# HunterJ-Lin/WSOVOD

Hardware: AMD Instinct MI355X
Metric: images/sec (512 proposals/img) WSR_18_DC5 fwd+bwd at 1/2/4/8 MI355X (higher is better)
Workload: dtype bf16 / fp16 + MX fp8 (the parity forward with the res4 / res5 convs and fc1 / fc2 on fp16 hi*hi + block-scaled e4m3 cross terms -- two v_mfma_f32_32x32x16_f16 + one v_mfma_scale_f32_32x32x64_f8f6f4 per 32x32x32 tile --, bf16x2 three-product forward elsewhere; plain bf16 backward; fp32 accumulation

## Files before the change

### include/wsovod_hip.h

```cpp
#ifndef WSOVOD_HIP_H_
#define WSOVOD_HIP_H_

#ifdef __cplusplus
extern "C" {
#endif

typedef void* wsovod_stream_t;

typedef enum {
  WSOVOD_OK = 0,
  WSOVOD_ERR_INVALID_ARGUMENT = 1,
  WSOVOD_ERR_HIP = 2,
  WSOVOD_ERR_UNSUPPORTED = 3
} wsovod_status;

typedef enum { WSOVOD_F32 = 0, WSOVOD_BF16 = 1, WSOVOD_BF16X2 = 2, WSOVOD_BF16X2P = 3, WSOVOD_F16MX = 4 } wsovod_dtype;
typedef enum { WSOVOD_NCHW = 0, WSOVOD_NHWC = 1 } wsovod_layout;

const char* wsovod_last_error(void);
int wsovod_abi_version(void);

typedef struct {
  const char* name;
  long long launches;
// ... 248 lines not shown

int wsovod_mask_transpose(const void* dy, long long lddy, const void* y, long long ldy, int in_dtype,
                          int M, int N, float scale, void* dA, long long ldda, void* dAt, long long ldt,
                          int out_dtype, wsovod_stream_t stream);
int wsovod_mask_transpose_colsum(const void* dy, long long lddy, const void* y, long long ldy, int in_dtype,
                                 int M, int N, float scale, void* dA, long long ldda, void* dAt, long long ldt,
                                 int out_dtype, float* colsum, wsovod_stream_t stream);
int wsovod_mask_transpose_ex(const void* dy, long long lddy, int dy_dtype, const void* y, long long ldy, int y_dtype, int M,
                             int N, float scale, void* dA, long long ldda, void* dAt, long long ldt, int out_dtype,
                             float* colsum, wsovod_stream_t stream);
int wsovod_bf16x2_encode(const float* src, long long ld_src, int rows, int cols, void* dst, long long ld_dst,
                         wsovod_stream_t stream);
int wsovod_bf16x2_decode(const void* src, long long ld_src, int rows, int cols, float* dst, long long ld_dst,
                         wsovod_stream_t stream);
int wsovod_mask_bf16x2(const float* dy, long long lddy, const void* y, long long ldy, int y_dtype, int M, int N, float scale,
                       void* dA_x2, long long ld_x2, void* dA_hi, long long ld_hi, float* colsum, wsovod_stream_t stream);
int wsovod_bf16x2_encode_t(const float* src, long long ld_src, int N, int K, void* dst, long long ld_dst,
                           wsovod_stream_t stream);
int wsovod_f16mx_to_f32(const void* src, long long ld_src, int rows, int cols, float* dst, long long ld_dst,
                        wsovod_stream_t stream);
int wsovod_f16mx_range(const void* src, long long ld, int rows, int cols, long long* counters, wsovod_stream_t stream);
int wsovod_stem_conv1_x2(const unsigned char* img, const int* sizes, const float* mean_host, const float* std_host, int N,
                         int Hp, int Wp, const void* w32x2, const float* bias, void* out, wsovod_stream_t stream);
int wsovod_add_group_rows(const void* x, long long ldx, int dtype, const int* row_group, const float* add,
                          long long ld_add, int M, int N, void* out, long long ldo, wsovod_stream_t stream);
int wsovod_scale_rows(const float* x, long long ldx, const float* row_scale, int R, int C, void* out,
                      long long ldo, int out_dtype, wsovod_stream_t stream);

int wsovod_data_aware_forward(const float* gap, int N, int C, const float* W1, const float* b1, int Hd,
                              const float* W2, const float* b2, int P, const float* E, int F, float* h1,
                              float* h2, float* daf, wsovod_stream_t stream);
int wsovod_data_aware_backward(const float* ddaf, int N, const float* gap, int C, const float* W2,
                               const float* E, int F, const float* h1, int Hd, const float* h2, int P,
                               float* dW1, float* db1, float* dW2, float* db2, float* dE,
                               float* scratch , wsovod_stream_t stream);

#ifdef __cplusplus
}
#endif
#endif
```

### wsovod_amd/_lib.py

```python
import ctypes as C
import os

import torch

_HERE = os.path.dirname(os.path.abspath(__file__))
LIB_PATH = os.path.join(_HERE, "lib", "libwsovod_hip.so")

F32, BF16, BF16X2, BF16X2P, F16MX = 0, 1, 2, 3, 4
NCHW, NHWC = 0, 1


class ConvGeom(C.Structure):
    _fields_ = [(n, C.c_int) for n in
                ("n_img", "H", "W", "Cin", "Ho", "Wo", "KH", "KW", "stride", "pad", "dil", "pool")]


class GemmDesc(C.Structure):
    _fields_ = [
        ("dtype_in", C.c_int), ("M", C.c_int), ("N", C.c_int), ("K", C.c_int),
        ("A", C.c_void_p), ("lda", C.c_longlong),
        ("B", C.c_void_p), ("ldb", C.c_longlong),
        ("C", C.c_void_p), ("ldc", C.c_longlong), ("dtype_c", C.c_int),
        ("Ct", C.c_void_p), ("ldct", C.c_longlong), ("dtype_ct", C.c_int),
        ("alpha", C.c_float),
# ... 21 lines not shown
_P, _I, _L, _F = C.c_void_p, C.c_int, C.c_longlong, C.c_float
ABI_VERSION = 9

SIGNATURES = {
    "wsovod_last_error": [],
    "wsovod_abi_version": [],
    "wsovod_profile_enable": [_I],
    "wsovod_profile_reset": [],
    "wsovod_profile_collect": [C.POINTER(ProfEntry), _I],
    "wsovod_roi_pool_forward": [_P, _I, _I, _P, _P, _I, _I, _I, _I, _I, _I, _I, _F, _P, _I, _P, _P],
    "wsovod_roi_pool_forward_x2hi": [_P, _I, _I, _P, _P, _I, _I, _I, _I, _I, _I, _I, _F, _P, _I, _P, _P, _P],
    "wsovod_roi_align_forward_x2hi": [_P, _I, _I, _P, _P, _I, _I, _I, _I, _I, _I, _I, _F, _I, _I, _P, _I, _P, _P],
    "wsovod_roi_pool_backward": [_P, _P, _P, _P, _I, _I, _I, _I, _I, _I, _I, _I, _P, _P],
    "wsovod_roi_loop_pool_forward": [_P, _I, _I, _P, _I, _I, _I, _I, _I, _I, _I, _F, _F, _P, _P, _P],
    "wsovod_roi_align_forward": [_P, _I, _I, _P, _P, _I, _I, _I, _I, _I, _I, _I, _F, _I, _I, _P, _I, _P],
    "wsovod_roi_align_backward": [_P, _P, _P, _I, _I, _I, _I, _I, _I, _I, _F, _I, _I, _I, _P, _P],
    "wsovod_gemm_nt": [C.POINTER(GemmDesc), _P],
    "wsovod_preprocess_image": [_P, _P, _P, _P, _I, _I, _I, _P, _P],
    "wsovod_stem_im2col": [_P, _P, _P, _P, _I, _I, _I, _P, _I, _P],
    "wsovod_stem_conv1": [_P, _P, _P, _P, _I, _I, _I, _P, _P, _P, _P],
    "wsovod_stem_im2col_ex": [_P, _P, _P, _P, _I, _I, _I, _I, _P, _I, _P],
    "wsovod_stem_conv1_s1": [_P, _P, _P, _P, _I, _I, _I, _P, _P, _P, _P],
    "wsovod_stem_conv1_s1_x2": [_P, _P, _P, _P, _I, _I, _I, _P, _P, _P, _P],
    "wsovod_maxpool2x2_nhwc": [_P, _I, _I, _I, _I, _I, _I, _I, _P, _P],
    "wsovod_maxpool2x2_nhwc_backward": [_P, _I, _I, _I, _I, _I, _I, _I, _P, _P, _P],
    "wsovod_global_avgpool_nhwc": [_P, _I, _I, _I, _I, _P, _P, _P],
    "wsovod_transpose_cast": [_P, _I, _L, _I, _I, _P, _I, _L, _P],
    "wsovod_cast": [_P, _I, _P, _I, _L, _P],
    "wsovod_row_l2norm_scale": [_P, _I, _L, _I, _I, _F, _F, _P, _P],
    "wsovod_row_l2norm_backward": [_P, _I, _L, _P, _L, _I, _I, _F, _F, _I, _P, _L, _P],
    "wsovod_segment_colsum": [_P, _I, _L, _P, _I, _I, _I, _P, _L, _I, _P, _P],
    "wsovod_colsum_workspace_floats": [_I, _I, _I],
    "wsovod_scale_by_device_scalar": [_P, _L, _P, _P, _P],
    "wsovod_sgd_momentum": [_P, _P, _P, _L, _F, _F, _F, _F, _P, _P],
    "wsovod_mil_forward": [_P, _L, _P, _I, _I, _P, _P, _P, _I, _P],
    "wsovod_mil_backward": [_P, _P, _P, _P, _I, _I, _P, _L, _I, _P],
    "wsovod_image_bce_forward": [_P, _P, _I, _I, _P, _F, _P, _P, _P, _P],
    "wsovod_image_bce_backward": [_P, _P, _I, _I, _P, _P, _P],
    "wsovod_weighted_ce_forward": [_P, _L, _I, _I, _P, _P, _I, _P, _L, _P, _P, _P],
    "wsovod_weighted_l1_box_forward": [_P, _L, _P, _P, _P, _P, _I, _I, _P, _F, _I, _P, _P, _P, _P, _P],
    "wsovod_mask_transpose": [_P, _L, _P, _L, _I, _I, _I, _F, _P, _L, _P, _L, _I, _P],
    "wsovod_mask_transpose_colsum": [_P, _L, _P, _L, _I, _I, _I, _F, _P, _L, _P, _L, _I, _P, _P],
    "wsovod_add_group_rows": [_P, _L, _I, _P, _P, _L, _I, _I, _P, _L, _P],
    "wsovod_scale_rows": [_P, _L, _P, _I, _I, _P, _L, _I, _P],
    "wsovod_data_aware_forward": [_P, _I, _I, _P, _P, _I, _P, _P, _I, _P, _I, _P, _P, _P, _P],
    "wsovod_data_aware_backward": [_P, _I, _P, _I, _P, _P, _I, _P, _I, _P, _I, _P, _P, _P, _P, _P, _P, _P],
# ... 134 lines not shown
```

### wsovod_amd/csrc/gemm.hip

```cpp
#include "gemm_common.h"
#include <type_traits>

namespace wsovod_gemm {

template <typename T, int BM, int BN, bool CONV, int WM = 2, int WN = 2, bool DMA = false, int STAGES = 2, bool X3 = false>
__global__ __launch_bounds__(64 * WM * WN) void gemm_nt_kernel(const GemmArgs p) {
  static_assert(!X3 || sizeof(T) == 2, "X3 is a bf16 variant");
  static_assert(!X3 || STAGES == 2 || DMA, "the deep X3 pipeline stages by LDS-DMA");
  constexpr int EPC = Traits<T>::EPC;
  constexpr int BKE = Traits<T>::BKE;
  constexpr int NT = 64 * WM * WN;
  constexpr int TM = BM / (WM * 16);
  constexpr int TN = BN / (WN * 16);
  constexpr int LR = NT / 8;
  constexpr int RA = BM / LR;
  constexpr int RB = BN / LR;
  static_assert(BM % LR == 0 && BN % LR == 0, "tile rows must be a multiple of the loader pass");
  extern __shared__ __attribute__((aligned(16))) char smem[];
  char* sA = smem;
  char* sB = smem + STAGES * BM * 128;

  const int nwg = p.tiles_m * p.tiles_n;
  int wg;
  {
// ... 1386 lines not shown
          acc[i][j] = __builtin_amdgcn_mfma_f32_16x16x32_bf16(__builtin_bit_cast(bf16x8, bl[j]),
                                                              __builtin_bit_cast(bf16x8, ah[i]), acc[i][j], 0, 0, 0);
#pragma unroll
      for (int i = 0; i < NI; ++i)
#pragma unroll
        for (int j = 0; j < 4; ++j)
          acc[i][j] = __builtin_amdgcn_mfma_f32_16x16x32_bf16(__builtin_bit_cast(bf16x8, bh[j]),
                                                              __builtin_bit_cast(bf16x8, al[i]), acc[i][j], 0, 0, 0);
    }
    __syncthreads();
  }
  c64x_epilogue<XG, NI>(p, acc, bias4, img, y0, x0, wave, frow, fq);
}

struct C64XH {
  static constexpr int TW = 32, XG = 2, NI = 4;
  static constexpr int PW = TW + 2, NPIX = PW * C64_PH;
  static constexpr int NPIX_PAD = (NPIX + 31) / 32 * 32;
  static constexpr int PATCH_BYTES = NPIX_PAD * 128;
  static constexpr int W_BYTES = 64 * 128;
  static constexpr int LDS_BYTES = PATCH_BYTES + 2 * W_BYTES;
};

template <bool LEPI>
__global__ __launch_bounds__(256, 2) void conv3x3_c64_x3h_kernel(const GemmArgs p, int tiles_x, int tiles_y) {
  using G = C64XH;
  constexpr int XG = G::XG, NI = G::NI, PW = G::PW;
  extern __shared__ __attribute__((aligned(16))) char smem[];
  char* sP = smem;
  char* sW = smem + G::PATCH_BYTES;
  const int tid = threadIdx.x, lane = tid & 63, wave = tid >> 6;
  const int tpi = tiles_x * tiles_y;
  const int img = blockIdx.x / tpi;
  const int t = blockIdx.x - img * tpi;
  const int ty = t / tiles_x, tx = t - ty * tiles_x;
  const int y0 = ty * C64_TH, x0 = tx * G::TW;
  typedef __attribute__((ext_vector_type(4))) unsigned int u32x4;
  [[maybe_unused]] const __amdgpu_buffer_rsrc_t rsrcA =
      __builtin_amdgcn_make_buffer_rsrc((void*)p.A, 0, (int)p.a_bytes, 0x00020000);
  [[maybe_unused]] const __amdgpu_buffer_rsrc_t rsrcB =
      __builtin_amdgcn_make_buffer_rsrc((void*)p.B, 0, (int)(64 * p.ldb * 2), 0x00020000);
  [[maybe_unused]] const int wave_u = __builtin_amdgcn_readfirstlane(wave);
  typedef __attribute__((address_space(3))) void lds_void [[maybe_unused]];

  auto stage_weights = [&](int step, int buf) {
#if defined(__HIP_DEVICE_COMPILE__)
    const int half = step >= 9 ? 1 : 0, tap = step - 9 * half;
#pragma unroll
// ... 6 lines not shown
                                               off, 0, 0, 0);
    }
#endif
  };
  auto stage_patch = [&](int half) {
#if defined(__HIP_DEVICE_COMPILE__)
    for (int base = 0; base < G::NPIX_PAD; base += 32) {
      const int q = base + wave_u * 8 + (lane >> 3);
      const int py = q / PW, px = q - py * PW;
      const int y = y0 - 1 + py, x = x0 - 1 + px;
      const bool ok = q < G::NPIX && y >= 0 && y < p.H && x >= 0 && x < p.W;
      const int chunk = (lane & 7) ^ ((q >> 1) & 7);
      const int off = (((img * p.H + y) * p.W + x) * 128 + half * 64 + chunk * 8) * 2;
      __builtin_amdgcn_raw_ptr_buffer_load_lds(rsrcA, (lds_void*)(sP + (base + wave_u * 8) * 128), 16, ok ? off : -1, 0, 0, 0);
    }
#endif
  };
#if C64XH_PHASES
  long long tph[6] = {0, 0, 0, 0, 0, 0}, tmark = (long long)__builtin_amdgcn_s_memtime();
#define C64XH_MARK(K) do { const long long n_ = (long long)__builtin_amdgcn_s_memtime(); tph[K] += n_ - tmark; tmark = n_; } while (0)
#else
#define C64XH_MARK(K) (void)0
#endif
  stage_patch(0);
  stage_weights(0, 0);
  stage_weights(1, 1);

  const int frow = lane & 15, fq = lane >> 4;
  f32x4 acc[NI][4];
#pragma unroll
  for (int i = 0; i < NI; ++i)
#pragma unroll
    for (int j = 0; j < 4; ++j) acc[i][j] = f32x4{0.f, 0.f, 0.f, 0.f};
  int qb[NI], boff[4];
#pragma unroll
  for (int i = 0; i < NI; ++i) qb[i] = (wave * 2 + (i / XG)) * PW + (i % XG) * 16 + frow;
#pragma unroll
  for (int j = 0; j < 4; ++j) {
    const int row = j * 16 + frow;
    boff[j] = row * 128 + ((fq ^ ((row >> 1) & 7)) << 4);
  }
  auto read_a = [&](int step, u32x4 (&ah)[NI], u32x4 (&al)[NI]) {
    const int tap = step >= 9 ? step - 9 : step;
    const int r = tap / 3;
    const int d = r * PW + (tap - r * 3);
#pragma unroll
    for (int i = 0; i < NI; ++i) {
      const int q = qb[i] + d;
      const int off = q * 128 + ((fq ^ ((q >> 1) & 7)) << 4);
// ... 25 lines not shown
#pragma unroll
    for (int i = 0; i < NI; ++i)
#pragma unroll
      for (int j = 0; j < 4; ++j)
        acc[i][j] = __builtin_amdgcn_mfma_f32_16x16x32_bf16(__builtin_bit_cast(bf16x8, bh[j]),
                                                            __builtin_bit_cast(bf16x8, al[i]), acc[i][j], 0, 0, 0);
  };
#define C64XH_INTERLEAVE(N)                                   \
  do {                                                        \
    _Pragma("unroll") for (int g_ = 0; g_ < (N); ++g_) {      \
      __builtin_amdgcn_sched_group_barrier(0x100, 1, 0);      \
      __builtin_amdgcn_sched_group_barrier(0x008, 3, 0);      \
    }                                                         \
  } while (0)
  u32x4 ah0[NI], al0[NI], bh0[4], bl0[4], ah1[NI], al1[NI], bh1[4], bl1[4];
  __syncthreads();
  read_a(0, ah0, al0);
  read_b(0, bh0, bl0);
  __syncthreads();
  C64XH_MARK(0);
  auto trip = [&](const int step, auto mode) {
    constexpr int MODE = decltype(mode)::value;
    if constexpr (MODE != 2) stage_weights(step + 2, 0);
    if constexpr (MODE == 1) stage_patch(1);
    read_b(step + 1, bh1, bl1);
    if constexpr (MODE != 1) read_a(step + 1, ah1, al1);
    mfma(ah0, al0, bh0, bl0);
    if constexpr (MODE != 1) C64XH_INTERLEAVE(16);
    else C64XH_INTERLEAVE(8);
    __builtin_amdgcn_sched_barrier(0);
    C64XH_MARK(2);
    __syncthreads();
    __builtin_amdgcn_sched_barrier(0);
    C64XH_MARK(3);
    if constexpr (MODE == 1) {
      read_a(9, ah1, al1);
      __builtin_amdgcn_sched_barrier(0);
    }
    if constexpr (MODE != 2) {
      stage_weights(step + 3, 1);
      read_b(step + 2, bh0, bl0);
      read_a(step + 2, ah0, al0);
    }
    mfma(ah1, al1, bh1, bl1);
    if constexpr (MODE != 2) C64XH_INTERLEAVE(16);
    __builtin_amdgcn_sched_barrier(0);
    C64XH_MARK(2);
// ... 1 lines not shown
    __builtin_amdgcn_sched_barrier(0);
    C64XH_MARK(3);
  };
#pragma unroll 1
  for (int step = 0; step < 8; step += 2) trip(step, std::integral_constant<int, 0>{});
  trip(8, std::integral_constant<int, 1>{});
#pragma unroll 1
  for (int step = 10; step < 16; step += 2) trip(step, std::integral_constant<int, 0>{});
  trip(16, std::integral_constant<int, 2>{});
  f32x4 bias4[4];
  c64_load_bias(p, fq, bias4);
  c64x_epilogue<XG, NI>(p, acc, bias4, img, y0, x0, wave, frow, fq, LEPI ? sP + wave_u * 4096 : nullptr);
#if C64XH_PHASES
  asm volatile("s_waitcnt vmcnt(0)" ::: "memory");
  C64XH_MARK(5);
  if (p.partial && tid == 0) {
    float* dst = p.partial + (blockIdx.x & 511) * 8;
    for (int k = 0; k < 6; ++k) atomicAdd(dst + k, (float)tph[k]);
    atomicAdd(dst + 7, 1.f);
  }
#endif
#undef C64XH_MARK
#undef C64XH_INTERLEAVE
}

template <typename T, int BM, int BN, bool CONV, int WM = 2, int WN = 2, bool DMA = false, int STAGES = 2, bool X3 = false>
int launch(const GemmArgs& a, hipStream_t s, const char* slot_name, double flops, double bytes) {
  static int slot = wsovod::prof_slot(slot_name);
  static bool attr_set = false;
  constexpr int lds_bytes = STAGES * (BM + BN) * 128;
  auto kfn = gemm_nt_kernel<T, BM, BN, CONV, WM, WN, DMA, STAGES, X3>;
  if (!attr_set) {
    WS_CHECK_HIP(hipFuncSetAttribute((const void*)kfn, hipFuncAttributeMaxDynamicSharedMemorySize, lds_bytes), "wsovod_gemm_nt: LDS opt-in");
    attr_set = true;
  }
  GemmArgs args = a;
  args.tiles_m = ceil_div(a.M - a.m_base, BM);
  args.tiles_n = ceil_div(a.N, BN);
  {
    const int run = std::max(1, args.tiles_m * args.tiles_n / 8);
    int g = 1;
    while ((g + 1) * (g + 1) <= run) ++g;
    args.group_m = std::max(1, std::min(g, args.tiles_m));
  }
  wsovod::ProfScope prof(slot, s, flops, bytes);
  hipLaunchKernelGGL(kfn, dim3(args.tiles_m * args.tiles_n), dim3(64 * WM * WN), lds_bytes, s, args);
// ... 360 lines not shown
      else if (d->K >= 2048 && (!d->conv || (cs && cs[0] == '1'))) tile = 2256256;
    }
    if (!d->tile_hint && d->conv && d->N > 64 && d->N <= 128 && (long long)ceil_div(d->M, 512) >= 200 &&
        !(getenv("WSOVOD_CONV_512") && getenv("WSOVOD_CONV_512")[0] == '0'))
      tile = 512128;
    if (!d->tile_hint && d->conv && getenv("WSOVOD_CONV_SPLITK") && getenv("WSOVOD_CONV_SPLITK")[0] == '1' && d->M >= 256 &&
        d->N >= 256 && d->K >= 2048 && (long long)ceil_div(d->M, 256) * ceil_div(d->N, 256) <= 128)
      tile = 2256256;
    static const bool deep = !(getenv("WSOVOD_X2_DEEP") && getenv("WSOVOD_X2_DEEP")[0] == '0');
    if (!d->tile_hint && deep) {
      if (tile == 1128064) tile = 3128064;
      else if (tile == 64064 && d->conv && d->K >= 1024 && d->M >= 1024) tile = 3064064;
    }
    if (planar) {
      WS_CHECK_ARG(!d->tile_hint || d->tile_hint == 2256256, "wsovod_gemm_nt: a planar A operand takes tile 2256256 only");
      tile = 2256256;
    }
    return d->conv ? dispatch_tile_x3<true>(a, tile, s, flops, bytes) : dispatch_tile_x3<false>(a, tile, s, flops, bytes);
  }
  if (d->dtype_in == WSOVOD_BF16)
    return d->conv ? dispatch_tile<bf16_t, true>(a, tile, s, flops, bytes) : dispatch_tile<bf16_t, false>(a, tile, s, flops, bytes);
  return d->conv ? dispatch_tile<float, true>(a, tile, s, flops, bytes) : dispatch_tile<float, false>(a, tile, s, flops, bytes);
}
```

### wsovod_amd/csrc/stem.hip

```cpp
#include "common.h"

namespace {

constexpr int S_TH = 8, S_TW = 32;
constexpr int S_PR = 2 * S_TH + 1, S_PC = 2 * S_TW + 1;
constexpr int S_PCP = S_PC + 1;

template <bool X2>
__device__ __forceinline__ void stem_stage_patch(const uint8_t* __restrict__ plane, int Hp, int Wp, int hi, int wi,
                                                 int y0, int x0, float m0, float m1, float m2, float s0, float s1,
                                                 float s2, bf16_t* lut_hi, bf16_t* lut_lo, bf16_t* patch_hi,
                                                 bf16_t* patch_lo) {
  const int tid = threadIdx.x, lane = tid & 63, wave = tid >> 6;
  for (int e = tid; e < 768; e += 256) {
    const int c = e >> 8;
    const float mean = c == 0 ? m0 : (c == 1 ? m1 : m2), sd = c == 0 ? s0 : (c == 1 ? s1 : s2);
    const float v = ((float)(e & 255) - mean) / sd;
    const bf16_t vh = (bf16_t)v;
    lut_hi[e] = vh;
    if (X2) lut_lo[e] = (bf16_t)(v - (float)vh);
  }
  __syncthreads();
  const bf16_t zero = (bf16_t)0.f;
  constexpr int RPW = (3 * S_PR + 3) / 4;
  const int w = 2 * x0 - 1 + lane, wc = min(max(w, 0), Wp - 1);
  const bool wok = w >= 0 && w < wi;
  const int w64 = 2 * x0 - 1 + 64, w64c = min(w64, Wp - 1);
  int byte[RPW + 1];
#pragma unroll
  for (int k = 0; k < RPW; ++k) {
    const int cr = min(wave + 4 * k, 3 * S_PR - 1);
    const int c = cr / S_PR, row = cr - c * S_PR;
    const int h = min(max(2 * y0 - 1 + row, 0), Hp - 1);
    byte[k] = plane[((long long)c * Hp + h) * Wp + wc];
  }
  {
    const int cr = min(tid, 3 * S_PR - 1), c = cr / S_PR, row = cr - c * S_PR;
    const int h = min(max(2 * y0 - 1 + row, 0), Hp - 1);
    byte[RPW] = plane[((long long)c * Hp + h) * Wp + w64c];
  }
// ... 21 lines not shown

__global__ __launch_bounds__(256) void stem_conv1_kernel(const uint8_t* __restrict__ img, const int* __restrict__ sizes,
                                                         float m0, float m1, float m2, float s0, float s1, float s2,
                                                         int N, int Hp, int Wp, int Ho, int Wo, int tiles_x, int tiles_y,
                                                         const bf16_t* __restrict__ w32, const float* __restrict__ bias,
                                                         bf16_t* __restrict__ out) {
  __shared__ bf16_t patch[3 * S_PR * S_PCP];
  const int tid = threadIdx.x, lane = tid & 63, wave = tid >> 6;
  const int frow = lane & 15, g = lane >> 4;
  const int tpi = tiles_x * tiles_y;
  const int n = blockIdx.x / tpi;
  const int t_in = blockIdx.x - n * tpi;
  const int ty = t_in / tiles_x, tx = t_in - ty * tiles_x;
  const int y0 = ty * S_TH, x0 = tx * S_TW;
  const int hi = sizes[2 * n], wi = sizes[2 * n + 1];
  const uint8_t* plane = img + (long long)n * 3 * Hp * Wp;
  __shared__ bf16_t lut[768];
  stem_stage_patch<false>(plane, Hp, Wp, hi, wi, y0, x0, m0, m1, m2, s0, s1, s2, lut, nullptr, patch, nullptr);
  bf16x8 bw[4];
#pragma unroll
  for (int j = 0; j < 4; ++j) bw[j] = *(const bf16x8*)(w32 + (16 * (frow >> 2) + 4 * j + (frow & 3)) * 32 + g * 8);
  int toff[8];
  bool real[8];
#pragma unroll
  for (int t = 0; t < 8; ++t) {
    const int k = 8 * g + t;
    const int tap = k / 3, c = k - 3 * tap, r = tap / 3, q = tap - 3 * r;
    real[t] = k < 27;
    toff[t] = real[t] ? (c * S_PR + r) * S_PCP + q : 0;
  }
  __syncthreads();
  const bf16_t zero = (bf16_t)0.f;
  f32x4 acc[4][4];
#pragma unroll
  for (int i = 0; i < 4; ++i) {
    const int ly = wave * 2 + (i >> 1), lx = (i & 1) * 16 + frow;
    const bf16_t* pb = patch + (2 * ly) * S_PCP + 2 * lx;
    bf16x8 a;
#pragma unroll
    for (int t = 0; t < 8; ++t) a[t] = real[t] ? pb[toff[t]] : zero;
#pragma unroll
    for (int j = 0; j < 4; ++j)
      acc[i][j] = __builtin_amdgcn_mfma_f32_16x16x32_bf16(bw[j], a, f32x4{0.f, 0.f, 0.f, 0.f}, 0, 0, 0);
  }
  f32x4 b4[4];
#pragma unroll
  for (int j = 0; j < 4; ++j) b4[j] = *(const f32x4*)(bias + 16 * g + 4 * j);
#pragma unroll
  for (int i = 0; i < 4; ++i) {
    const int y = y0 + wave * 2 + (i >> 1), x = x0 + (i & 1) * 16 + frow;
    if (y >= Ho || x >= Wo) continue;
    bf16x8 lo, hi8;
#pragma unroll
// ... 16 lines not shown
                                                            bf16_t* __restrict__ out) {
  __shared__ bf16_t patch_hi[3 * S_PR * S_PCP];
  __shared__ bf16_t patch_lo[3 * S_PR * S_PCP];
  const int tid = threadIdx.x, lane = tid & 63, wave = tid >> 6;
  const int frow = lane & 15, g = lane >> 4;
  const int tpi = tiles_x * tiles_y;
  const int n = blockIdx.x / tpi;
  const int t_in = blockIdx.x - n * tpi;
  const int ty = t_in / tiles_x, tx = t_in - ty * tiles_x;
  const int y0 = ty * S_TH, x0 = tx * S_TW;
  const int hi = sizes[2 * n], wi = sizes[2 * n + 1];
  const uint8_t* plane = img + (long long)n * 3 * Hp * Wp;
  __shared__ bf16_t lut_hi[768], lut_lo[768];
  stem_stage_patch<true>(plane, Hp, Wp, hi, wi, y0, x0, m0, m1, m2, s0, s1, s2, lut_hi, lut_lo, patch_hi, patch_lo);
  bf16x8 bwh[4], bwl[4];
#pragma unroll
  for (int j = 0; j < 4; ++j) {
    const bf16_t* wr = w32x2 + (16 * (frow >> 2) + 4 * j + (frow & 3)) * 64 + g * 8;
    bwh[j] = *(const bf16x8*)wr;
    bwl[j] = *(const bf16x8*)(wr + 32);
  }
  int toff[8];
  bool real[8];
#pragma unroll
  for (int t = 0; t < 8; ++t) {
    const int k = 8 * g + t;
    const int tap = k / 3, c = k - 3 * tap, r = tap / 3, q = tap - 3 * r;
    real[t] = k < 27;
    toff[t] = real[t] ? (c * S_PR + r) * S_PCP + q : 0;
  }
  __syncthreads();
  const bf16_t zero = (bf16_t)0.f;
  f32x4 acc[4][4];
#pragma unroll
  for (int i = 0; i < 4; ++i) {
    const int ly = wave * 2 + (i >> 1), lx = (i & 1) * 16 + frow;
    const int po = (2 * ly) * S_PCP + 2 * lx;
    bf16x8 ah, al;
#pragma unroll
    for (int t = 0; t < 8; ++t) {
      ah[t] = real[t] ? patch_hi[po + toff[t]] : zero;
      al[t] = real[t] ? patch_lo[po + toff[t]] : zero;
    }
#pragma unroll
    for (int j = 0; j < 4; ++j) {
      f32x4 c4 = __builtin_amdgcn_mfma_f32_16x16x32_bf16(bwh[j], ah, f32x4{0.f, 0.f, 0.f, 0.f}, 0, 0, 0);
      c4 = __builtin_amdgcn_mfma_f32_16x16x32_bf16(bwl[j], ah, c4, 0, 0, 0);
      acc[i][j] = __builtin_amdgcn_mfma_f32_16x16x32_bf16(bwh[j], al, c4, 0, 0, 0);
    }
  }
  f32x4 b4[4];
#pragma unroll
  for (int j = 0; j < 4; ++j) b4[j] = *(const f32x4*)(bias + 16 * g + 4 * j);
#pragma unroll
  for (int i = 0; i < 4; ++i) {
    const int y = y0 + wave * 2 + (i >> 1), x = x0 + (i & 1) * 16 + frow;
    if (y >= Ho || x >= Wo) continue;
    bf16x8 h0, h1, l0, l1;
#pragma unroll
    for (int r = 0; r < 4; ++r) {
      const float v0 = fmaxf(acc[i][0][r] + b4[0][r], 0.f), v1 = fmaxf(acc[i][1][r] + b4[1][r], 0.f);
      const float v2 = fmaxf(acc[i][2][r] + b4[2][r], 0.f), v3 = fmaxf(acc[i][3][r] + b4[3][r], 0.f);
      h0[r] = (bf16_t)v0; h0[4 + r] = (bf16_t)v1; h1[r] = (bf16_t)v2; h1[4 + r] = (bf16_t)v3;
      l0[r] = (bf16_t)(v0 - (float)h0[r]); l0[4 + r] = (bf16_t)(v1 - (float)h0[4 + r]);
      l1[r] = (bf16_t)(v2 - (float)h1[r]); l1[4 + r] = (bf16_t)(v3 - (float)h1[4 + r]);
    }
    bf16_t* dst = out + (((long long)n * Ho + y) * Wo + x) * 128 + 64 * (g >> 1) + 16 * (g & 1);
    *(bf16x8*)dst = h0;
    *(bf16x8*)(dst + 8) = h1;
    *(bf16x8*)(dst + 32) = l0;
    *(bf16x8*)(dst + 40) = l1;
  }
}

constexpr int S1_PR = S_TH + 2, S1_PC = S_TW + 2;
constexpr int S1_PCP = S1_PC + 2;

template <bool X2>
__device__ __forceinline__ void stem_stage_patch_s1(const uint8_t* __restrict__ plane, int Hp, int Wp, int hi, int wi,
                                                    int y0, int x0, float m0, float m1, float m2, float s0, float s1,
                                                    float s2, bf16_t* lut_hi, bf16_t* lut_lo, bf16_t* patch_hi,
                                                    bf16_t* patch_lo) {
  const int tid = threadIdx.x, lane = tid & 63, wave = tid >> 6;
  for (int e = tid; e < 768; e += 256) {
    const int c = e >> 8;
    const float mean = c == 0 ? m0 : (c == 1 ? m1 : m2), sd = c == 0 ? s0 : (c == 1 ? s1 : s2);
    const float v = ((float)(e & 255) - mean) / sd;
    const bf16_t vh = (bf16_t)v;
    lut_hi[e] = vh;
    if (X2) lut_lo[e] = (bf16_t)(v - (float)vh);
  }
  __syncthreads();
  const bf16_t zero = (bf16_t)0.f;
  constexpr int ROWS = 3 * S1_PR, RPW = (ROWS + 3) / 4;
  const int w = x0 - 1 + lane, wc = min(max(w, 0), Wp - 1);
  const bool wok = w >= 0 && w < wi;
  int byte[RPW];
#pragma unroll
  for (int k = 0; k < RPW; ++k) {
    const int cr = min(wave + 4 * k, ROWS - 1);
    const int c = cr / S1_PR, row = cr - c * S1_PR;
    const int h = min(max(y0 - 1 + row, 0), Hp - 1);
    byte[k] = plane[((long long)c * Hp + h) * Wp + wc];
  }
#pragma unroll
  for (int k = 0; k < RPW; ++k) {
    const int cr = wave + 4 * k;
    if (cr < ROWS && lane < S1_PC) {
      const int c = cr / S1_PR, row = cr - c * S1_PR;
      const int h = y0 - 1 + row;
// ... 14 lines not shown
  __shared__ bf16_t patch_hi[3 * S1_PR * S1_PCP];
  __shared__ bf16_t patch_lo[X2 ? 3 * S1_PR * S1_PCP : 1];
  __shared__ bf16_t lut_hi[768], lut_lo[X2 ? 768 : 1];
  const int tid = threadIdx.x, lane = tid & 63, wave = tid >> 6;
  const int frow = lane & 15, g = lane >> 4;
  const int tpi = tiles_x * tiles_y;
  const int n = blockIdx.x / tpi;
  const int t_in = blockIdx.x - n * tpi;
  const int ty = t_in / tiles_x, tx = t_in - ty * tiles_x;
  const int y0 = ty * S_TH, x0 = tx * S_TW;
  const int hi = sizes[2 * n], wi = sizes[2 * n + 1];
  const uint8_t* plane = img + (long long)n * 3 * Hp * Wp;
  stem_stage_patch_s1<X2>(plane, Hp, Wp, hi, wi, y0, x0, m0, m1, m2, s0, s1, s2, lut_hi, lut_lo, patch_hi, patch_lo);
  constexpr int WLD = X2 ? 64 : 32;
  bf16x8 bwh[4], bwl[4];
#pragma unroll
  for (int j = 0; j < 4; ++j) {
    const bf16_t* wr = wq + (16 * (frow >> 2) + 4 * j + (frow & 3)) * WLD + g * 8;
    bwh[j] = *(const bf16x8*)wr;
    if (X2) bwl[j] = *(const bf16x8*)(wr + 32);
  }
  int toff[8];
  bool real[8];
#pragma unroll
  for (int t = 0; t < 8; ++t) {
    const int k = 8 * g + t;
    const int tap = k / 3, c = k - 3 * tap, r = tap / 3, q = tap - 3 * r;
    real[t] = k < 27;
    toff[t] = real[t] ? (c * S1_PR + r) * S1_PCP + q : 0;
  }
  __syncthreads();
  const bf16_t zero = (bf16_t)0.f;
  f32x4 acc[4][4];
#pragma unroll
  for (int i = 0; i < 4; ++i) {
    const int ly = wave * 2 + (i >> 1), lx = (i & 1) * 16 + frow;
    const int po = ly * S1_PCP + lx;
    bf16x8 ah, al;
#pragma unroll
    for (int t = 0; t < 8; ++t) {
      ah[t] = real[t] ? patch_hi[po + toff[t]] : zero;
      if (X2) al[t] = real[t] ? patch_lo[po + toff[t]] : zero;
    }
#pragma unroll
    for (int j = 0; j < 4; ++j) {
      f32x4 c4 = __builtin_amdgcn_mfma_f32_16x16x32_bf16(bwh[j], ah, f32x4{0.f, 0.f, 0.f, 0.f}, 0, 0, 0);
      if (X2) {
        c4 = __builtin_amdgcn_mfma_f32_16x16x32_bf16(bwl[j], ah, c4, 0, 0, 0);
        c4 = __builtin_amdgcn_mfma_f32_16x16x32_bf16(bwh[j], al, c4, 0, 0, 0);
      }
      acc[i][j] = c4;
    }
  }
// ... 117 lines not shown
```

### wsovod_amd/layers/hip_ops.py

```python
import ctypes as C
import contextlib
import os
import threading

import torch

from .. import _lib
from .._lib import BF16, BF16X2, BF16X2P, F16MX, F32, NCHW, NHWC, GemmDesc, check, dtype_code, lib, ptr, require_gpu, stream
from . import carrier, operand_cache


_CONST_CACHE = {}


class _ConstOverride(threading.local):
    table = None


_OVERRIDE = _ConstOverride()


class const_override:
    def __init__(self, table):
        self.table = table
# ... 474 lines not shown
def x2_encode_t(src):
    require_gpu(src)
    carrier.refuse("x2_encode_t", (src,))
    if src.dtype != torch.float32 or src.dim() != 2 or src.stride(1) != 1:
        raise RuntimeError("x2_encode_t: source must be a 2-D fp32 matrix with a contiguous last dim")
    N, K = src.shape
    out = torch.empty((K, (N + 31) // 32 * 32), dtype=torch.float32, device=src.device)
    check(lib().wsovod_bf16x2_encode_t(ptr(src), src.stride(0), N, K, ptr(out), out.stride(0), stream()), "bf16x2_encode_t")
    return carrier.tag(out, X2)


def x2t_cached(t):
    return operand_cache.lookup(t, "x2t", x2_encode_t)


def stem_conv1_x2(images_u8, sizes, mean, std, w32_x2, bias):
    require_gpu(images_u8, sizes, w32_x2, bias)
    assert w32_x2.dtype == torch.float32 and tuple(w32_x2.shape) == (64, 32) and w32_x2.is_contiguous()
    N, _, Hp, Wp = images_u8.shape
    Ho, Wo = (Hp - 1) // 2 + 1, (Wp - 1) // 2 + 1
    out = torch.empty((N, Ho, Wo, 64), dtype=torch.float32, device=images_u8.device)
    check(lib().wsovod_stem_conv1_x2(ptr(images_u8), ptr(sizes), _f3(mean), _f3(std), N, Hp, Wp, ptr(w32_x2), ptr(bias),
                                     ptr(out), stream()), "stem_conv1_x2")
    return carrier.tag(out, X2)


import threading


class _X3StateT(threading.local):
    active = False


_X3State = _X3StateT()


class x3_mode:

    def __init__(self, on=True):
        self.on = ("full" if on is True else on) if on else False

    def __enter__(self):
        self.prev = _X3State.active
        _X3State.active = self.on
        return self

# ... 786 lines not shown
```

### wsovod_amd/modeling/backbone.py

```python
import os
import warnings

import numpy as np
import torch
import torch.nn.functional as F
from torch import nn

from ..config import BACKBONE_REGISTRY
from ..layers import carrier, hip_ops as H, mx_guard
from ..structures import ShapeSpec

__all__ = ["BasicStem", "BasicBlock", "BottleneckBlock", "ResNet", "FrozenForwardMixin", "FrozenBatchNorm2d", "Conv2d",
           "build_wsl_resnet_backbone", "make_stage"]


class FrozenBatchNorm2d(nn.Module):

    def __init__(self, num_features, eps=1e-5):
        super().__init__()
        self.num_features = num_features
        self.eps = eps
        self.register_buffer("weight", torch.ones(num_features))
        self.register_buffer("bias", torch.zeros(num_features))
        self.register_buffer("running_mean", torch.zeros(num_features))
# ... 246 lines not shown
        self.conv2 = Conv2d(out_channels, out_channels, 3, stride=1, padding=1, bias=False,
                            norm=get_norm(norm, out_channels))
        self.conv3 = Conv2d(out_channels, out_channels, 3, stride=1, padding=1, bias=False,
                            norm=get_norm(norm, out_channels))
        for c in (self.conv1, self.conv2, self.conv3):
            c2_msra_fill(c)

    def _tail(self, x):
        x = hip_conv(x, self.conv2, relu=True)
        return hip_conv(x, self.conv3, relu=True, pool2=True)

    def forward(self, x):
        return self._tail(hip_conv(x, self.conv1, relu=True))

    def _im2col_weight(self, dtype):
        wq, b = self.conv1.folded(dtype)
        wpad = getattr(self, "_w_im2col", None)
        if wpad is None or wpad[0] is not wq:
            w32 = torch.zeros((wq.size(0), 32), dtype=wq.dtype, device=wq.device)
            w32[:, :27] = wq
            self._w_im2col = wpad = (wq, w32)
        return wpad[1], b

    def forward_uint8(self, images_u8, sizes, pixel_mean, pixel_std):
        if _x2():
            w32, b = self._im2col_weight(torch.float32)
            return self._tail(H.stem_conv1_x2(images_u8, sizes, pixel_mean, pixel_std, H.x2_cached(w32), b))
        w32, b = self._im2col_weight(torch.bfloat16)
        return self._tail(H.stem_conv1(images_u8, sizes, pixel_mean, pixel_std, w32, b))

    def forward_im2col(self, a, n, ho, wo):
        assert self.in_channels == 3
        wq, b = self.conv1.folded(a.dtype)
        wpad = getattr(self, "_w_im2col", None)
        if wpad is None or wpad[0] is not wq:
            w32 = torch.zeros((wq.size(0), 32), dtype=wq.dtype, device=wq.device)
            w32[:, :27] = wq
            self._w_im2col = wpad = (wq, w32)
        x = H.gemm_nt(a, wpad[1], bias=b, relu=True, out_dtype=a.dtype).view(n, ho, wo, self.out_channels)
        return self._tail(x)


def _torch_conv(conv, x):
    y = F.conv2d(x, conv.weight, conv.bias, conv.stride, conv.padding, conv.dilation)
    if conv.norm is not None:
        scale, shift = conv.norm.scale_shift()
        y = y * scale.view(1, -1, 1, 1) + shift.view(1, -1, 1, 1)
    return y

# ... 568 lines not shown
```

Measured before the change: 1429.

## Fuse stem conv1 into the conv2 3x3 c64 kernel, computing patches on the fly

Adds a fused stem kernel that normalises uint8 image pixels through a LUT and computes conv1 (bf16x2, three-product) directly into the LDS patch of the conv3x3_c64_x3h kernel, which then runs conv2. This removes the conv1 output write and re-read through global memory and one launch on the x2 forward path. The second half of the patch is computed mid-loop in place of the async patch stage. The cost is recomputation of halo pixels, more LDS per workgroup, and extra ALU work inside the conv2 pipeline. Shared stem helpers are factored into a common header.

```diff
diff --git a/include/wsovod_hip.h b/include/wsovod_hip.h
--- a/include/wsovod_hip.h
+++ b/include/wsovod_hip.h
@@ -294,6 +294,9 @@
 int wsovod_f16mx_range(const void* src, long long ld, int rows, int cols, long long* counters, wsovod_stream_t stream);
 int wsovod_stem_conv1_x2(const unsigned char* img, const int* sizes, const float* mean_host, const float* std_host, int N,
                          int Hp, int Wp, const void* w32x2, const float* bias, void* out, wsovod_stream_t stream);
+int wsovod_stem_conv12_x2(const unsigned char* img, const int* sizes, const float* mean_host, const float* std_host, int N,
+                          int Hp, int Wp, const void* w32x2, const float* bias1, const void* w2x2, const float* bias2,
+                          void* out, wsovod_stream_t stream);
 int wsovod_add_group_rows(const void* x, long long ldx, int dtype, const int* row_group, const float* add,
                           long long ld_add, int M, int N, void* out, long long ldo, wsovod_stream_t stream);
 int wsovod_scale_rows(const float* x, long long ldx, const float* row_scale, int R, int C, void* out,
diff --git a/wsovod_amd/_lib.py b/wsovod_amd/_lib.py
--- a/wsovod_amd/_lib.py
+++ b/wsovod_amd/_lib.py
@@ -67,6 +67,7 @@
     "wsovod_stem_im2col_ex": [_P, _P, _P, _P, _I, _I, _I, _I, _P, _I, _P],
     "wsovod_stem_conv1_s1": [_P, _P, _P, _P, _I, _I, _I, _P, _P, _P, _P],
     "wsovod_stem_conv1_s1_x2": [_P, _P, _P, _P, _I, _I, _I, _P, _P, _P, _P],
+    "wsovod_stem_conv12_x2": [_P, _P, _P, _P, _I, _I, _I, _P, _P, _P, _P, _P, _P],
     "wsovod_maxpool2x2_nhwc": [_P, _I, _I, _I, _I, _I, _I, _I, _P, _P],
     "wsovod_maxpool2x2_nhwc_backward": [_P, _I, _I, _I, _I, _I, _I, _I, _P, _P, _P],
     "wsovod_global_avgpool_nhwc": [_P, _I, _I, _I, _I, _P, _P, _P],
diff --git a/wsovod_amd/csrc/gemm.hip b/wsovod_amd/csrc/gemm.hip
--- a/wsovod_amd/csrc/gemm.hip
+++ b/wsovod_amd/csrc/gemm.hip
@@ -1,4 +1,5 @@
 #include "gemm_common.h"
+#include "stem_common.h"
 #include <type_traits>
 
 namespace wsovod_gemm {
@@ -1432,8 +1433,18 @@
   static constexpr int LDS_BYTES = PATCH_BYTES + 2 * W_BYTES;
 };
 
-template <bool LEPI>
-__global__ __launch_bounds__(256, 2) void conv3x3_c64_x3h_kernel(const GemmArgs p, int tiles_x, int tiles_y) {
+struct C64XH_STEM {
+  static constexpr int SR = 2 * C64_PH + 1, SC = 2 * C64XH::PW + 1;
+  static constexpr int SCP = SC + 1;
+  static constexpr int U_BYTES = 3 * SR * SCP * 4;
+  static constexpr int LDS_BYTES = C64XH::LDS_BYTES + U_BYTES;
+  static_assert(2 * LDS_BYTES <= 160 * 1024, "conv3x3_c64_x3h_stem_kernel: two workgroups per CU");
+  static_assert(768 * 4 <= C64XH::PATCH_BYTES, "the normalisation table lies in the patch region");
+};
+
+template <bool LEPI, bool STEM>
+__device__ __forceinline__ void conv3x3_c64_x3h_body(const GemmArgs& p, const wsovod_stem::StemSrc& st, const int tiles_x,
+                                                     const int tiles_y) {
   using G = C64XH;
   constexpr int XG = G::XG, NI = G::NI, PW = G::PW;
   extern __shared__ __attribute__((aligned(16))) char smem[];
@@ -1486,9 +1497,112 @@
 #else
 #define C64XH_MARK(K) (void)0
 #endif
-  stage_patch(0);
-  stage_weights(0, 0);
-  stage_weights(1, 1);
+  [[maybe_unused]] unsigned* sU = (unsigned*)(smem + G::LDS_BYTES);
+  [[maybe_unused]] auto stem_stage = [&]() {
+    using S = C64XH_STEM;
+    unsigned* sLut = (unsigned*)sP;
+    for (int e = tid; e < 768; e += 256) {
+      const float v = wsovod_stem::lut_value(e, st.m0, st.m1, st.m2, st.s0, st.s1, st.s2);
+      const bf16_t vh = (bf16_t)v, vl = (bf16_t)(v - (float)vh);
+      sLut[e] = (unsigned)__builtin_bit_cast(unsigned short, vh) | ((unsigned)__builtin_bit_cast(unsigned short, vl) << 16);
+    }
+    const int hi = st.sizes[2 * img], wi = st.sizes[2 * img + 1];
+    const uint8_t* plane = st.img + (long long)img * 3 * st.Hp * st.Wp;
+    constexpr int LINES = 3 * S::SR, LPW = (LINES + 3) / 4, XC = S::SC - 64, XT = (LINES * XC + 255) / 256;
+    const int w = 2 * x0 - 3 + lane, wc = min(max(w, 0), st.Wp - 1);
+    const bool wok = w >= 0 && w < wi;
+    int byte[LPW + XT];
+#pragma unroll
+    for (int k = 0; k < LPW; ++k) {
+      const int cr = min(wave + 4 * k, LINES - 1), c = cr / S::SR, row = cr - c * S::SR;
+      const int h = min(max(2 * y0 - 3 + row, 0), st.Hp - 1);
+      byte[k] = plane[((long long)c * st.Hp + h) * st.Wp + wc];
+    }
+#pragma unroll
+    for (int k = 0; k < XT; ++k) {
+      const int e = min(tid + 256 * k, LINES * XC - 1), cr = e / XC, col = 64 + (e - cr * XC);
+      const int c = cr / S::SR, row = cr - c * S::SR;
+      const int h = min(max(2 * y0 - 3 + row, 0), st.Hp - 1), wx = min(2 * x0 - 3 + col, st.Wp - 1);
+      byte[LPW + k] = plane[((long long)c * st.Hp + h) * st.Wp + wx];
+    }
+    __syncthreads();
+#pragma unroll
+    for (int k = 0; k < LPW; ++k) {
+      const int cr = wave + 4 * k;
+      if (cr < LINES) {
+        const int c = cr / S::SR, row = cr - c * S::SR, h = 2 * y0 - 3 + row;
+        const bool ok = h >= 0 && h < hi && wok;
+        sU[cr * S::SCP + lane] = ok ? sLut[c * 256 + byte[k]] : 0u;
+      }
+    }
+#pragma unroll
+    for (int k = 0; k < XT; ++k) {
+      const int e = tid + 256 * k;
+      if (e < LINES * XC) {
+        const int cr = e / XC, col = 64 + (e - cr * XC), c = cr / S::SR, row = cr - c * S::SR;
+        const int h = 2 * y0 - 3 + row, wx = 2 * x0 - 3 + col;
+        const bool ok = h >= 0 && h < hi && wx < wi;
+        sU[cr * S::SCP + col] = ok ? sLut[c * 256 + byte[LPW + k]] : 0u;
+      }
+    }
+    __syncthreads();
+  };
+  [[maybe_unused]] auto stem_half = [&](const int half) {
+    using S = C64XH_STEM;
+    const int prow = lane & 15, g = lane >> 4;
+    int toff[8];
+    bool real[8];
+    wsovod_stem::tap_offsets(g, S::SR, S::SCP, toff, real);
+    bf16x8 wh[2], wl[2];
+    f32x4 b4[2];
+#pragma unroll
+    for (int j = 0; j < 2; ++j) {
+      const bf16_t* wr = st.w32x2 + (32 * half + 8 * (prow >> 2) + 4 * j + (prow & 3)) * 64 + g * 8;
+      wh[j] = *(const bf16x8*)wr;
+      wl[j] = *(const bf16x8*)(wr + 32);
+      b4[j] = *(const f32x4*)(st.bias + 32 * half + 8 * g + 4 * j);
+    }
+#pragma unroll 1
+    for (int pg = wave_u; pg < G::NPIX_PAD / 16; pg += 4) {
+      const int q = pg * 16 + prow;
+      const int py = q / PW, px = q - py * PW;
+      const int y = y0 - 1 + py, x = x0 - 1 + px;
+      const bool ok = q < G::NPIX && y >= 0 && y < p.H && x >= 0 && x < p.W;
+      const int po = ok ? 2 * py * S::SCP + 2 * px : 0;
+      bf16x8 ah, al;
+#pragma unroll
+      for (int t = 0; t < 8; ++t) {
+        const unsigned u = real[t] ? sU[po + toff[t]] : 0u;
+        ah[t] = __builtin_bit_cast(bf16_t, (unsigned short)(u & 0xffffu));
+        al[t] = __builtin_bit_cast(bf16_t, (unsigned short)(u >> 16));
+      }
+      bf16x8 h8, l8;
+#pragma unroll
+      for (int j = 0; j < 2; ++j) {
+        const f32x4 c4 = wsovod_stem::mfma_x2(wh[j], wl[j], ah, al);
+#pragma unroll
+        for (int r = 0; r < 4; ++r) {
+          bf16_t h, l;
+          wsovod_stem::relu_split(c4[r], b4[j][r], h, l);
+          h8[4 * j + r] = ok ? h : (bf16_t)0.f;
+          l8[4 * j + r] = ok ? l : (bf16_t)0.f;
+        }
+      }
+      const int off = q * 128 + ((g ^ ((q >> 1) & 7)) << 4);
+      *(bf16x8*)(sP + off) = h8;
+      *(bf16x8*)(sP + (off ^ 64)) = l8;
+    }
+  };
+  if constexpr (STEM) {
+    stage_weights(0, 0);
+    stage_weights(1, 1);
+    stem_stage();
+    stem_half(0);
+  } else {
+    stage_patch(0);
+    stage_weights(0, 0);
+    stage_weights(1, 1);
+  }
 
   const int frow = lane & 15, fq = lane >> 4;
   f32x4 acc[NI][4];
@@ -1560,7 +1674,14 @@
   auto trip = [&](const int step, auto mode) {
     constexpr int MODE = decltype(mode)::value;
     if constexpr (MODE != 2) stage_weights(step + 2, 0);
-    if constexpr (MODE == 1) stage_patch(1);
+    if constexpr (MODE == 1) {
+      if constexpr (STEM) {
+        stem_half(1);
+        __builtin_amdgcn_sched_barrier(0);
+      } else {
+        stage_patch(1);
+      }
+    }
     read_b(step + 1, bh1, bl1);
     if constexpr (MODE != 1) read_a(step + 1, ah1, al1);
     mfma(ah0, al0, bh0, bl0);
@@ -1608,6 +1729,16 @@
 #endif
 #undef C64XH_MARK
 #undef C64XH_INTERLEAVE
+}
+
+template <bool LEPI>
+__global__ __launch_bounds__(256, 2) void conv3x3_c64_x3h_kernel(const GemmArgs p, int tiles_x, int tiles_y) {
+  conv3x3_c64_x3h_body<LEPI, false>(p, wsovod_stem::StemSrc{}, tiles_x, tiles_y);
+}
+
+__global__ __launch_bounds__(256, 2) void conv3x3_c64_x3h_stem_kernel(const GemmArgs p, const wsovod_stem::StemSrc st,
+                                                                      int tiles_x, int tiles_y) {
+  conv3x3_c64_x3h_body<true, true>(p, st, tiles_x, tiles_y);
 }
 
 template <typename T, int BM, int BN, bool CONV, int WM = 2, int WN = 2, bool DMA = false, int STAGES = 2, bool X3 = false>
@@ -2014,3 +2145,61 @@
     return d->conv ? dispatch_tile<bf16_t, true>(a, tile, s, flops, bytes) : dispatch_tile<bf16_t, false>(a, tile, s, flops, bytes);
   return d->conv ? dispatch_tile<float, true>(a, tile, s, flops, bytes) : dispatch_tile<float, false>(a, tile, s, flops, bytes);
 }
+
+extern "C" int wsovod_stem_conv12_x2(const unsigned char* img, const int* sizes, const float* mean_host,
+                                     const float* std_host, int N, int Hp, int Wp, const void* w32x2, const float* bias1,
+                                     const void* w2x2, const float* bias2, void* out, wsovod_stream_t stream) {
+  WS_CHECK_ARG(N >= 0 && Hp > 0 && Wp > 0, "wsovod_stem_conv12_x2: bad shape");
+  if (N == 0) return WSOVOD_OK;
+  WS_CHECK_ARG(img && sizes && mean_host && std_host && w32x2 && bias1 && w2x2 && bias2 && out,
+               "wsovod_stem_conv12_x2: null pointer");
+  WS_CHECK_ARG((((uintptr_t)w32x2 | (uintptr_t)bias1 | (uintptr_t)w2x2 | (uintptr_t)bias2 | (uintptr_t)out) & 15) == 0,
+               "wsovod_stem_conv12_x2: weights / biases / output must be 16-byte aligned");
+  const int Ho = (Hp - 1) / 2 + 1, Wo = (Wp - 1) / 2 + 1;
+  const long long total = (long long)N * Ho * Wo;
+  const int tiles_x = ceil_div(Wo, C64XH::TW), tiles_y = ceil_div(Ho, C64_TH);
+  if (total >= (1ll << 31) || (long long)N * tiles_x * tiles_y >= (1ll << 31)) {
+    wsovod::set_error("wsovod_stem_conv12_x2: %lld output pixels are more than one launch addresses", total);
+    return WSOVOD_ERR_UNSUPPORTED;
+  }
+  GemmArgs a;
+  memset(&a, 0, sizeof(a));
+  a.B = (const char*)w2x2;
+  a.ldb = 2 * 9 * 64;
+  a.M = (int)total;
+  a.N = 64;
+  a.K = 2 * 9 * 64;
+  a.C = out;
+  a.ldc = 64;
+  a.dtype_c = WSOVOD_BF16X2;
+  a.alpha = 1.f;
+  a.bias = bias2;
+  a.relu = 1;
+  a.H = a.Ho = Ho;
+  a.W = a.Wo = Wo;
+  a.Cin = 128;
+  a.KH = a.KW = 3;
+  a.stride = a.pad = a.dil = 1;
+  wsovod_stem::StemSrc st;
+  st.img = img;
+  st.sizes = sizes;
+  st.m0 = mean_host[0], st.m1 = mean_host[1], st.m2 = mean_host[2];
+  st.s0 = std_host[0], st.s1 = std_host[1], st.s2 = std_host[2];
+  st.Hp = Hp, st.Wp = Wp;
+  st.w32x2 = (const bf16_t*)w32x2;
+  st.bias = bias1;
+  static int slot = wsovod::prof_slot("stem_conv12_fused_bf16x2");
+  static bool attr = false;
+  if (!attr) {
+    WS_CHECK_HIP(hipFuncSetAttribute((const void*)conv3x3_c64_x3h_stem_kernel, hipFuncAttributeMaxDynamicSharedMemorySize,
+                                     C64XH_STEM::LDS_BYTES), "wsovod_stem_conv12_x2: LDS opt-in");
+    attr = true;
+  }
+  hipStream_t s = (hipStream_t)stream;
+  wsovod::ProfScope prof(slot, s, 6.0 * total * 64 * (9 * 64 + 27 * 340.0 / 256),
+                         (double)N * 3 * Hp * Wp + 64.0 * (9 * 64 + 32) * 4 + (double)total * 256);
+  hipLaunchKernelGGL(conv3x3_c64_x3h_stem_kernel, dim3((unsigned)(N * tiles_x * tiles_y)), dim3(256),
+                     C64XH_STEM::LDS_BYTES, s, a, st, tiles_x, tiles_y);
+  WS_CHECK_LAUNCH("wsovod_stem_conv12_x2");
+  return WSOVOD_OK;
+}
diff --git a/wsovod_amd/csrc/stem.hip b/wsovod_amd/csrc/stem.hip
--- a/wsovod_amd/csrc/stem.hip
+++ b/wsovod_amd/csrc/stem.hip
@@ -1,4 +1,5 @@
 #include "common.h"
+#include "stem_common.h"
 
 namespace {
 
@@ -13,9 +14,7 @@
                                                  bf16_t* patch_lo) {
   const int tid = threadIdx.x, lane = tid & 63, wave = tid >> 6;
   for (int e = tid; e < 768; e += 256) {
-    const int c = e >> 8;
-    const float mean = c == 0 ? m0 : (c == 1 ? m1 : m2), sd = c == 0 ? s0 : (c == 1 ? s1 : s2);
-    const float v = ((float)(e & 255) - mean) / sd;
+    const float v = wsovod_stem::lut_value(e, m0, m1, m2, s0, s1, s2);
     const bf16_t vh = (bf16_t)v;
     lut_hi[e] = vh;
     if (X2) lut_lo[e] = (bf16_t)(v - (float)vh);
@@ -83,13 +82,7 @@
   for (int j = 0; j < 4; ++j) bw[j] = *(const bf16x8*)(w32 + (16 * (frow >> 2) + 4 * j + (frow & 3)) * 32 + g * 8);
   int toff[8];
   bool real[8];
-#pragma unroll
-  for (int t = 0; t < 8; ++t) {
-    const int k = 8 * g + t;
-    const int tap = k / 3, c = k - 3 * tap, r = tap / 3, q = tap - 3 * r;
-    real[t] = k < 27;
-    toff[t] = real[t] ? (c * S_PR + r) * S_PCP + q : 0;
-  }
+  wsovod_stem::tap_offsets(g, S_PR, S_PCP, toff, real);
   __syncthreads();
   const bf16_t zero = (bf16_t)0.f;
   f32x4 acc[4][4];
@@ -152,13 +145,7 @@
   }
   int toff[8];
   bool real[8];
-#pragma unroll
-  for (int t = 0; t < 8; ++t) {
-    const int k = 8 * g + t;
-    const int tap = k / 3, c = k - 3 * tap, r = tap / 3, q = tap - 3 * r;
-    real[t] = k < 27;
-    toff[t] = real[t] ? (c * S_PR + r) * S_PCP + q : 0;
-  }
+  wsovod_stem::tap_offsets(g, S_PR, S_PCP, toff, real);
   __syncthreads();
   const bf16_t zero = (bf16_t)0.f;
   f32x4 acc[4][4];
@@ -173,11 +160,7 @@
       al[t] = real[t] ? patch_lo[po + toff[t]] : zero;
     }
 #pragma unroll
-    for (int j = 0; j < 4; ++j) {
-      f32x4 c4 = __builtin_amdgcn_mfma_f32_16x16x32_bf16(bwh[j], ah, f32x4{0.f, 0.f, 0.f, 0.f}, 0, 0, 0);
-      c4 = __builtin_amdgcn_mfma_f32_16x16x32_bf16(bwl[j], ah, c4, 0, 0, 0);
-      acc[i][j] = __builtin_amdgcn_mfma_f32_16x16x32_bf16(bwh[j], al, c4, 0, 0, 0);
-    }
+    for (int j = 0; j < 4; ++j) acc[i][j] = wsovod_stem::mfma_x2(bwh[j], bwl[j], ah, al);
   }
   f32x4 b4[4];
 #pragma unroll
@@ -189,11 +172,11 @@
     bf16x8 h0, h1, l0, l1;
 #pragma unroll
     for (int r = 0; r < 4; ++r) {
-      const float v0 = fmaxf(acc[i][0][r] + b4[0][r], 0.f), v1 = fmaxf(acc[i][1][r] + b4[1][r], 0.f);
-      const float v2 = fmaxf(acc[i][2][r] + b4[2][r], 0.f), v3 = fmaxf(acc[i][3][r] + b4[3][r], 0.f);
-      h0[r] = (bf16_t)v0; h0[4 + r] = (bf16_t)v1; h1[r] = (bf16_t)v2; h1[4 + r] = (bf16_t)v3;
-      l0[r] = (bf16_t)(v0 - (float)h0[r]); l0[4 + r] = (bf16_t)(v1 - (float)h0[4 + r]);
-      l1[r] = (bf16_t)(v2 - (float)h1[r]); l1[4 + r] = (bf16_t)(v3 - (float)h1[4 + r]);
+      bf16_t h, l;
+      wsovod_stem::relu_split(acc[i][0][r], b4[0][r], h, l); h0[r] = h; l0[r] = l;
+      wsovod_stem::relu_split(acc[i][1][r], b4[1][r], h, l); h0[4 + r] = h; l0[4 + r] = l;
+      wsovod_stem::relu_split(acc[i][2][r], b4[2][r], h, l); h1[r] = h; l1[r] = l;
+      wsovod_stem::relu_split(acc[i][3][r], b4[3][r], h, l); h1[4 + r] = h; l1[4 + r] = l;
     }
     bf16_t* dst = out + (((long long)n * Ho + y) * Wo + x) * 128 + 64 * (g >> 1) + 16 * (g & 1);
     *(bf16x8*)dst = h0;
@@ -213,9 +196,7 @@
                                                     bf16_t* patch_lo) {
   const int tid = threadIdx.x, lane = tid & 63, wave = tid >> 6;
   for (int e = tid; e < 768; e += 256) {
-    const int c = e >> 8;
-    const float mean = c == 0 ? m0 : (c == 1 ? m1 : m2), sd = c == 0 ? s0 : (c == 1 ? s1 : s2);
-    const float v = ((float)(e & 255) - mean) / sd;
+    const float v = wsovod_stem::lut_value(e, m0, m1, m2, s0, s1, s2);
     const bf16_t vh = (bf16_t)v;
     lut_hi[e] = vh;
     if (X2) lut_lo[e] = (bf16_t)(v - (float)vh);
@@ -276,13 +257,7 @@
   }
   int toff[8];
   bool real[8];
-#pragma unroll
-  for (int t = 0; t < 8; ++t) {
-    const int k = 8 * g + t;
-    const int tap = k / 3, c = k - 3 * tap, r = tap / 3, q = tap - 3 * r;
-    real[t] = k < 27;
-    toff[t] = real[t] ? (c * S1_PR + r) * S1_PCP + q : 0;
-  }
+  wsovod_stem::tap_offsets(g, S1_PR, S1_PCP, toff, real);
   __syncthreads();
   const bf16_t zero = (bf16_t)0.f;
   f32x4 acc[4][4];
diff --git a/wsovod_amd/csrc/stem_common.h b/wsovod_amd/csrc/stem_common.h
--- /dev/null
+++ b/wsovod_amd/csrc/stem_common.h
@@ -0,0 +1,44 @@
+#pragma once
+#include "common.h"
+
+namespace wsovod_stem {
+
+__device__ __forceinline__ float lut_value(const int e, const float m0, const float m1, const float m2, const float s0,
+                                           const float s1, const float s2) {
+  const int c = e >> 8;
+  const float mean = c == 0 ? m0 : (c == 1 ? m1 : m2), sd = c == 0 ? s0 : (c == 1 ? s1 : s2);
+  return ((float)(e & 255) - mean) / sd;
+}
+
+__device__ __forceinline__ void tap_offsets(const int g, const int rows, const int pcp, int (&toff)[8], bool (&real)[8]) {
+#pragma unroll
+  for (int t = 0; t < 8; ++t) {
+    const int k = 8 * g + t;
+    const int tap = k / 3, c = k - 3 * tap, r = tap / 3, q = tap - 3 * r;
+    real[t] = k < 27;
+    toff[t] = real[t] ? (c * rows + r) * pcp + q : 0;
+  }
+}
+
+__device__ __forceinline__ f32x4 mfma_x2(const bf16x8 wh, const bf16x8 wl, const bf16x8 ah, const bf16x8 al) {
+  f32x4 c4 = __builtin_amdgcn_mfma_f32_16x16x32_bf16(wh, ah, f32x4{0.f, 0.f, 0.f, 0.f}, 0, 0, 0);
+  c4 = __builtin_amdgcn_mfma_f32_16x16x32_bf16(wl, ah, c4, 0, 0, 0);
+  return __builtin_amdgcn_mfma_f32_16x16x32_bf16(wh, al, c4, 0, 0, 0);
+}
+
+__device__ __forceinline__ void relu_split(const float acc, const float bias, bf16_t& hi, bf16_t& lo) {
+  const float v = fmaxf(acc + bias, 0.f);
+  hi = (bf16_t)v;
+  lo = (bf16_t)(v - (float)hi);
+}
+
+struct StemSrc {
+  const uint8_t* img;
+  const int* sizes;
+  float m0, m1, m2, s0, s1, s2;
+  int Hp, Wp;
+  const bf16_t* w32x2;
+  const float* bias;
+};
+
+}
diff --git a/wsovod_amd/layers/hip_ops.py b/wsovod_amd/layers/hip_ops.py
--- a/wsovod_amd/layers/hip_ops.py
+++ b/wsovod_amd/layers/hip_ops.py
@@ -520,6 +520,30 @@
     out = torch.empty((N, Ho, Wo, 64), dtype=torch.float32, device=images_u8.device)
     check(lib().wsovod_stem_conv1_x2(ptr(images_u8), ptr(sizes), _f3(mean), _f3(std), N, Hp, Wp, ptr(w32_x2), ptr(bias),
                                      ptr(out), stream()), "stem_conv1_x2")
+    return carrier.tag(out, X2)
+
+
+STEM_CONV12_MAX_PIXELS = (1 << 31) - 1
+
+
+def stem_conv12_x2_takes(images_u8):
+    N, _, Hp, Wp = images_u8.shape
+    if any(os.environ.get(k) is not None for k in ("WSOVOD_C64X_TW", "WSOVOD_C64_X3", "WSOVOD_C64X_LEPI")):
+        return False
+    return 0 < N * ((Hp - 1) // 2 + 1) * ((Wp - 1) // 2 + 1) <= STEM_CONV12_MAX_PIXELS
+
+
+def stem_conv12_x2(images_u8, sizes, mean, std, w32_x2, bias1, w2_x2, bias2):
+    require_gpu(images_u8, sizes, w32_x2, bias1, w2_x2, bias2)
+    carrier.refuse("stem_conv12_x2", (w32_x2, w2_x2))
+    assert w32_x2.dtype == torch.float32 and tuple(w32_x2.shape) == (64, 32) and w32_x2.is_contiguous()
+    assert w2_x2.dtype == torch.float32 and tuple(w2_x2.shape) == (64, 9 * 64) and w2_x2.is_contiguous()
+    assert bias1.dtype == torch.float32 and bias2.dtype == torch.float32 and bias1.numel() == 64 and bias2.numel() == 64
+    N, _, Hp, Wp = images_u8.shape
+    Ho, Wo = (Hp - 1) // 2 + 1, (Wp - 1) // 2 + 1
+    out = torch.empty((N, Ho, Wo, 64), dtype=torch.float32, device=images_u8.device)
+    check(lib().wsovod_stem_conv12_x2(ptr(images_u8), ptr(sizes), _f3(mean), _f3(std), N, Hp, Wp, ptr(w32_x2), ptr(bias1),
+                                      ptr(w2_x2), ptr(bias2), ptr(out), stream()), "stem_conv12_x2")
     return carrier.tag(out, X2)
 
 
diff --git a/wsovod_amd/modeling/backbone.py b/wsovod_amd/modeling/backbone.py
--- a/wsovod_amd/modeling/backbone.py
+++ b/wsovod_amd/modeling/backbone.py
@@ -292,9 +292,21 @@
             self._w_im2col = wpad = (wq, w32)
         return wpad[1], b
 
+    def _fuses_conv1(self, images_u8):
+        if os.environ.get("WSOVOD_FUSE_STEM", "1") == "0":
+            return False
+        c2 = self.conv2
+        return (self.in_channels == 3 and self.out_channels == 64 and c2.out_channels == 64
+                and (c2.kernel_size, c2.stride, c2.padding, c2.dilation) == (3, 1, 1, 1)
+                and H.stem_conv12_x2_takes(images_u8))
+
     def forward_uint8(self, images_u8, sizes, pixel_mean, pixel_std):
         if _x2():
             w32, b = self._im2col_weight(torch.float32)
+            if self._fuses_conv1(images_u8):
+                w2, b2 = _folded_x2(self.conv2, cin_pad=64)
+                x = H.stem_conv12_x2(images_u8, sizes, pixel_mean, pixel_std, H.x2_cached(w32), b, w2, b2)
+                return hip_conv(x, self.conv3, relu=True, pool2=True)
             return self._tail(H.stem_conv1_x2(images_u8, sizes, pixel_mean, pixel_std, H.x2_cached(w32), b))
         w32, b = self._im2col_weight(torch.bfloat16)
         return self._tail(H.stem_conv1(images_u8, sizes, pixel_mean, pixel_std, w32, b))
```

Result: no change. 1441 (median of 6 runs) (+0.8%).
